# TinyMPC/tinympc-matlab

Hardware: AMD Instinct MI355X
Metric: ADMM iterations/s, batched quadrotor nx=12 nu=4 N=50 (instance-iterations/s, whole job) (higher is better)
Workload: dtype f64

## Files before the change

### __graft_entry__.py

```python
from __future__ import annotations

import hashlib
import importlib.util
import os
import re
import shutil
import subprocess
import sys

ROOT = os.path.dirname(os.path.abspath(__file__))
if ROOT not in sys.path:
    sys.path.insert(0, ROOT)
PKG_DIR = os.path.join(ROOT, "tinympc-matlab_amd")
PKG_NAME = "tinympc_matlab_amd"
CSRC = os.path.join(PKG_DIR, "csrc")
HIP_LIB = os.path.join(PKG_DIR, "libtinympc_hip.so")
ORACLE_DIR = os.path.join(ROOT, "oracle")
REFERENCE_SRC = "/root/reference/src/codegen_src"

HIP_SOURCES = ["tinympc_kernels.hip", "tinympc_precompute_rows.hip", "tinympc_solve.hip", "tinympc_solve_b.hip", "tinympc_solve_fam.hip", "tinympc_solve_adapt.hip", "tinympc_imod_a.hip", "tinympc_ifam_a.hip", "tinympc_solve_c.hip", "tinympc_solve_d.hip", "tinympc_solve_dr.hip", "tinympc_lean_d.hip", "tinympc_lstart_d.hip", "tinympc_ltrim_d.hip", "tinympc_lshare_d.hip", "tinympc_solve_dw.hip", "tinympc_solve_dx.hip", "tinympc_jit.hip", "tinympc_solve_m.hip", "tinympc_precompute_large.hip", "tinympc_handle.hip", "tinympc_plan.hip", "tinympc_session.hip", "tinympc_capi.hip",
               "tinympc_codegen.hip"]
HIP_LINTED = ["tinympc_precompute_rows.hip", "tinympc_solve.hip", "tinympc_solve_b.hip", "tinympc_solve_fam.hip", "tinympc_solve_adapt.hip", "tinympc_imod_a.hip", "tinympc_ifam_a.hip",
              "tinympc_solve_c.hip", "tinympc_solve_d.hip", "tinympc_solve_dr.hip", "tinympc_lean_d.hip", "tinympc_lstart_d.hip", "tinympc_ltrim_d.hip", "tinympc_lshare_d.hip", "tinympc_solve_dw.hip", "tinympc_solve_dx.hip"]
JIT_EMBEDDED = ["tinympc_device.h", "tinympc_sweep.h", "tinympc_fam_red.h", "tinympc_solve_d_chain.h", "tinympc_solve_dw_chain.h", "tinympc_solve_dx_chain.h",
                "tinympc_solve_e_common.h", "tinympc_solve_dwide.h", "tinympc_solve_d.hip", "tinympc_solve_dw.hip", "tinympc_solve_dx.hip", "tinympc_solve_e.hip",
                "tinympc_solve_f.hip"]
_ROCKET = ["-DTINY_JIT_NX=6", "-DTINY_JIT_NU=3", "-DTINY_JIT_N=100", "-DTINY_JIT_CT=0", "-DTINY_JIT_FAM=1"]
_ROCKET_FAM = ["-DTINY_JIT_E_NROUND=1", "-DTINY_JIT_E_NCONE=2", "-DTINY_JIT_E_CONES={0,0,2},{0,6,8}", "-DTINY_JIT_E_NLX=1", "-DTINY_JIT_E_NLU=0"]
HIP_BUILTINS = [
    ("k_builtin_e_rocket100", "tinympc_solve_e.hip",
     _ROCKET + ["-DTINY_JIT_E_WPG=8", "-DTINY_JIT_E_WPS=2", "-DTINY_JIT_E_S=13"] + _ROCKET_FAM +
     ["-DTINY_JIT_E_GC_LDS=0", "-DTINY_JIT_E_GL_LDS=0", "-DTINY_JIT_E_LX_LDS=0", "-DTINY_JIT_E_KFAM=1", "-DTINY_JIT_E_DREG=1"]),
    ("k_builtin_f_rocket100", "tinympc_solve_f.hip", _ROCKET + ["-DTINY_JIT_F_WPG=4", "-DTINY_JIT_F_S=7"] + _ROCKET_FAM + ["-DTINY_JIT_F_KFAM=1"]),
    ("k_builtin_f_rocket100_session", "tinympc_solve_f.hip", _ROCKET + ["-DTINY_JIT_F_WPG=4", "-DTINY_JIT_F_S=7"] + _ROCKET_FAM + ["-DTINY_JIT_F_KFAM=1", "-DTINY_JIT_F_SESSION=1"]),
]
_NO_FAM = ["-DTINY_JIT_E_NROUND=0", "-DTINY_JIT_E_NCONE=0", "-DTINY_JIT_E_CONES={-1,0,0}", "-DTINY_JIT_E_NLX=0", "-DTINY_JIT_E_NLU=0"]
for _name, _nx, _nu, _N, _wpg, _S in (("cartpole20", 4, 1, 20, 2, 3), ("quadrotor50", 12, 4, 50, 4, 4)):
    for _suffix, _ct, _extra in (("", 1, []), ("_var", 0, []), ("_session", 0, ["-DTINY_JIT_F_SESSION=1"])):
        HIP_BUILTINS.append(("k_builtin_f_%s%s" % (_name, _suffix), "tinympc_solve_f.hip",
                             ["-DTINY_JIT_NX=%d" % _nx, "-DTINY_JIT_NU=%d" % _nu, "-DTINY_JIT_N=%d" % _N, "-DTINY_JIT_CT=%d" % _ct, "-DTINY_JIT_FAM=0",
                              "-DTINY_JIT_F_WPG=%d" % _wpg, "-DTINY_JIT_F_S=%d" % _S] + _NO_FAM + _extra))
HIP_BUILTINS_D = [("k_builtin_d_quadrotor50_models", "tinympc_solve_d.hip",
                   ["-DTINY_JIT_NX=12", "-DTINY_JIT_NU=4", "-DTINY_JIT_N=50", "-DTINY_JIT_VREG=49", "-DTINY_JIT_WPS=1", "-DTINY_JIT_WPG=4",
                    "-DTINY_JIT_CT=1", "-DTINY_JIT_FAM=0", "-DTINY_JIT_ADAPT=0", "-DTINY_JIT_IMOD=1"]),
                  ("k_builtin_d_quadrotor20_lin1", "tinympc_solve_d.hip",
                   ["-DTINY_JIT_NX=12", "-DTINY_JIT_NU=4", "-DTINY_JIT_N=20", "-DTINY_JIT_VREG=19", "-DTINY_JIT_WPS=1", "-DTINY_JIT_WPG=4",
# ... 308 lines not shown
```

### tinympc-matlab_amd/csrc/tinympc_device.h

```cpp
#pragma once
#ifndef __HIPCC_RTC__
#include <hip/hip_runtime.h>
#endif

namespace tinympc {

__host__ __device__ inline size_t ops_doubles(int W, int KT) { return (size_t)2 * W * KT + 3 * W; }

__host__ __device__ inline size_t table_rows(int N) { return (size_t)N + 2; }

constexpr int V_PAD = 4;
__host__ __device__ inline size_t v_rows(int N) { return (size_t)N + 1 + 2 * V_PAD; }
__host__ __device__ inline size_t tables_doubles(int W, int N) { return 3 * table_rows(N) * W + W; }

#if defined(__HIPCC__) || defined(__HIPCC_RTC__)
__device__ __forceinline__ void host_store(double *p, double v) { __hip_atomic_store(p, v, __ATOMIC_RELAXED, __HIP_MEMORY_SCOPE_SYSTEM); }
#endif

struct PrecomputeParams {
    int nx, nu;
    union { double rho; const double *rho_sys; };
    const double *A, *B, *fdyn, *Qd, *Rd;
    double *Kinf, *Pinf, *Quu_inv, *AmBKt, *APf, *BPf;
    int *info;
// ... 294 lines not shown
hipError_t launch_build_inst_tables(const InstTableParams &p, hipStream_t stream);
hipError_t launch_fill_inst_models(const InstModelFillParams &p, hipStream_t stream);
hipError_t launch_store_inst_diag(const InstDiagParams &p, hipStream_t stream);
hipError_t launch_check_positive(const double *v, int n, int *flag, hipStream_t stream);
hipError_t launch_build_inst_lin(const InstLinParams &p, hipStream_t stream);
hipError_t launch_check_inst_lin(const InstLinParams &p, int *flag, hipStream_t stream);
hipError_t launch_check_inst_slopes(const InstSlopeParams &p, int *flag, hipStream_t stream);
hipError_t launch_store_inst_slopes(const InstSlopeParams &p, hipStream_t stream);
hipError_t launch_build_inst_slopes(const InstSlopeParams &p, hipStream_t stream);
hipError_t launch_check_ref_steps(const int *steps, int n, int delta, int *flag, hipStream_t stream);
hipError_t launch_advance_ref_steps(int *steps, int n, int delta, hipStream_t stream);
enum class SolveExt { Box, Families, Adaptive, InstRefs, InstBounds, InstModels, InstFamilies };
hipError_t launch_solve_a(const SolveParams &p, SolveExt ext, int W, int KT, size_t lds_bytes, hipStream_t stream);
hipError_t launch_solve_b(const SolveParams &p, int W, int KT, size_t lds_bytes, hipStream_t stream);
size_t solve_b_lds_bytes(int nx, int nu, int N, int W);
constexpr int WAVES_PER_GROUP_B = 4;
bool solve_d_supported(int nx, int nu, int N, bool const_tables);
hipError_t launch_solve_d(const SolveParams &p, hipStream_t stream);
hipError_t launch_solve_d_refill(const SolveParams &p, hipStream_t stream);
hipError_t launch_solve_d_lean(const SolveParams &p, hipStream_t stream);
hipError_t launch_solve_d_lean_start(const SolveParams &p, hipStream_t stream);
hipError_t launch_solve_d_lean_trim(const SolveParams &p, hipStream_t stream);
hipError_t launch_solve_d_lean_share(const SolveParams &p, hipStream_t stream);
int solve_d_workgroups(int nu, int N, bool const_tables, int groups);
size_t solve_d_lds_bytes(int nu, int N, bool const_tables);
int solve_d_resident_workgroups(int wpg);
int solve_d_wavefronts_per_workgroup(int nu, int N, bool const_tables);
bool solve_dw_supported(int nx, int nu, int N, bool const_tables);
hipError_t launch_solve_dw(const SolveParams &p, hipStream_t stream);
int solve_dw_workgroups(int nu, int N, int groups);
size_t solve_dw_lds_bytes(int nu, int N);
bool solve_dx_supported(int nx, int nu, int N, bool const_tables);
hipError_t launch_solve_dx(const SolveParams &p, hipStream_t stream);
int solve_dx_workgroups(int nu, int N, int groups);
size_t solve_dx_lds_bytes(int nu, int N);
hipError_t launch_solve_c(const SolveParams &p, int W, int KT, size_t lds_bytes, hipStream_t stream);
hipError_t launch_build_chunk_tables(const ChunkTableParams &p, hipStream_t stream);
size_t f_input_table_doubles(int nu, int S);
hipError_t launch_build_f_input_tables(const ChunkTableParams &p, hipStream_t stream);
void chunk_plan(int N, int *S, int *C, int *Lc);
size_t solve_c_lds_bytes(int nx, int Lc);
size_t solve_c_lds_bytes_refs(int nx, int nu, int N, int Lc);
size_t chunk_table_doubles(int nx, int Lc);
int chunk_ks(int nx);
hipError_t launch_build_adapt(const AdaptTableParams &p, hipStream_t stream);
inline hipError_t ensure_dynamic_lds(const void *fn, size_t bytes, size_t (&cache)[16]) {
// ... 42 lines not shown
```

### tinympc-matlab_amd/csrc/tinympc_plan.hip

```cpp
#include <cstring>
#include "tinympc_handle.h"

using namespace tinympc;
using namespace tinympc::host;

namespace {

void arm_completion_flag(tinympc_solver *s, SolveParams &p) {
    if (!p.host_sol) return;
    s->session_seq += 1;
    p.host_seq = (double)s->session_seq;
    s->flag_pending = true;
}

void decide_layout_d_variants(tinympc_solver *s) {
    if (!s->layout_d) return;
    if (s->d_varying < 0 && !s->tables_const()) {
        if (s->W == 16 && !s->d_jit && solve_d_supported(s->nx, s->nu, s->N, false)) {
            s->d_varying = 1;
        } else {
            s->d_varying_jit = solve_jit_supported(s->W, s->nx, s->nu, s->N, false);
            s->d_varying = s->d_varying_jit ? 1 : 0;
        }
    }
// ... 240 lines not shown
    if (pl.kernel != KernelId::D_COMPILED || s->W != 16 || pl.adaptive || pl.families || s->zero_copy_tick || s->st.max_iter <= 0)
        return false;
    if (pl.inst_models) return false;
    if (refill_applies(s, pl)) return false;
    const char *env = getenv("TINYMPC_LEAN");
    const int mode = env ? atoi(env) : -1;
    if (mode == 0) return false;
    if (mode == 1) return true;
    const bool reachable = s->st.abs_pri_tol > 0.0 && s->st.abs_dua_tol > 0.0;
    return s->st.check_termination != 1 || !reachable;
}
static bool lean_start_applies() {
    const char *env = getenv("TINYMPC_LEAN_START");
    return !env || atoi(env) != 0;
}
static bool lean_trim_applies() {
    const char *env = getenv("TINYMPC_LEAN_TRIM");
    return lean_start_applies() && (!env || atoi(env) != 0);
}
static bool lean_share_applies() {
    const char *env = getenv("TINYMPC_LEAN_SHARE");
    return lean_trim_applies() && (!env || atoi(env) != 0);
}
static const char *lean_words(const tinympc_solver *s, const LaunchPlan &pl) {
    return !lean_applies(s, pl)   ? ""
           : lean_share_applies() ? " lean lds-start trim share"
           : lean_trim_applies()  ? " lean lds-start trim"
           : lean_start_applies() ? " lean lds-start"
                                  : " lean";
}

int launch(tinympc_solver *s, bool timed) {
    int rc;
    s->flag_pending = false;
    if ((rc = resolve_plan(s))) return rc;
    const LaunchPlan pl = current_plan(s);
    const bool fam = pl.families, adaptive = pl.adaptive;
    if (s->inst.fam() && !pl.inst_lin) {
        const char *why = s->layout_m ? "for systems with nx+nu > 64"
                          : s->inst.models ? (s->inst.rho_verb ? "with per-instance models or rho (set_model_batch / set_rho_batch); tinympc_clear_model_batch returns to the shared model and rho"
                                                               : "with per-instance models (set_model_batch); tinympc_clear_model_batch returns to the shared model")
                          : adaptive ? "with adaptive rho"
                                     : "with more cones or rounds of overlapping cones than the generic kernel holds";
        if (!s->inst.lin)
            return fail(TINYMPC_ERR_UNSUPPORTED, "per-instance cone slopes (set_cone_slopes_batch) are not supported %s; "
                        "tinympc_set_cone_constraints returns to shared slopes", why);
        return fail(TINYMPC_ERR_UNSUPPORTED, "per-instance linear constraints (set_linear_constraints_batch)%s are not supported %s; "
                    "tinympc_set_linear_constraints returns to shared rows%s", s->inst.cones ? " and cone slopes (set_cone_slopes_batch)" : "", why,
// ... 97 lines not shown
    p.rho_min = s->st.adaptive_rho_min; p.rho_max = s->st.adaptive_rho_max; p.rho_clip = s->st.adaptive_rho_enable_clipping;
    const bool kernel_takes_cold = (pl.kernel == KernelId::D_COMPILED || pl.kernel == KernelId::D_JIT) && s->st.max_iter > 0;
    if (s->cold_state && !kernel_takes_cold && (rc = materialize_cold_state(s))) return rc;
    p.cold = s->cold_state ? 1 : 0;
    s->cold_state = false;
    if (s->st.max_iter > 0) s->sol_zero_pending = false;
    else if ((rc = materialize_zero_solution(s))) return rc;
    if (refill_applies(s, pl) && !p.x0_mirror && !p.u0_host && !p.host_sol) {
        if (!s->drefill && (rc = dalloc(s, &s->drefill, 1))) return rc;
        HIP_TRY(hipMemsetAsync(s->drefill, 0, sizeof(int), s->stream));
        p.refill_next = s->drefill;
    }
    if (timed) HIP_TRY(hipEventRecord(s->ev0, s->stream));
    switch (pl.kernel) {
        case KernelId::M:
            p.ctab = s->dctab;
            HIP_TRY(launch_solve_m(p, s->stream));
            break;
        case KernelId::D_JIT:
            HIP_TRY(launch_solve_jit(p, s->W, s->stream, pl.inst_models, pl.inst_lin ? s->ifam_nl() : 0, pl.inst_lin && s->inst.cones));
            break;
        case KernelId::D_COMPILED:
            if (lean_applies(s, pl) && !p.x0_mirror && !p.u0_host && !p.refill_next)
                HIP_TRY(lean_share_applies()   ? launch_solve_d_lean_share(p, s->stream)
                        : lean_trim_applies()  ? launch_solve_d_lean_trim(p, s->stream)
                        : lean_start_applies() ? launch_solve_d_lean_start(p, s->stream)
                                               : launch_solve_d_lean(p, s->stream));
            else HIP_TRY(s->W == 64 ? launch_solve_dx(p, s->stream) : s->W == 32 ? launch_solve_dw(p, s->stream) : launch_solve_d(p, s->stream));
            break;
        case KernelId::E:
            p.ctab = s->dctab_e; p.chunk_len = s->e_chunk_len; p.chunk_count = s->e_wpg; p.chunk_levels = 1;
            HIP_TRY(launch_solve_e(p, s->fs, s->stream));
            break;
        case KernelId::F:
            p.ctab = s->dctab_f; p.ftab = s->dftab; p.chunk_len = s->f_chunk_len; p.chunk_count = s->f_chunks; p.chunk_levels = 4;
            arm_completion_flag(s, p);
            HIP_TRY(launch_solve_f(p, s->f_fs, s->stream));
            break;
        case KernelId::C:
            p.ctab = s->dctab; p.chunk_len = s->chunk_len; p.chunk_count = s->chunk_count; p.chunk_levels = s->chunk_levels;
            arm_completion_flag(s, p);
            HIP_TRY(launch_solve_c(p, s->W, s->KT, s->lds_bytes_c, s->stream));
            break;
        case KernelId::B:
            HIP_TRY(launch_solve_b(p, s->W, s->KT, s->lds_bytes, s->stream));
            break;
        case KernelId::A:
// ... 107 lines not shown
```

### tinympc-matlab_amd/csrc/tinympc_solve_d.hip

```cpp
#if defined(TINY_BUILTIN) && !defined(TINY_JIT)
#define TINY_JIT 1
#endif
#ifndef TINY_JIT
#include <atomic>
#endif
#include <type_traits>

#include "tinympc_device.h"
#include "tinympc_sweep.h"

#ifndef TINY_REFILL
#if defined(TINY_JIT_REFILL) && TINY_JIT_REFILL
#define TINY_REFILL 1
#else
#define TINY_REFILL 0
#endif
#endif

#ifndef TINY_LEAN
#define TINY_LEAN 0
#endif
#if TINY_LEAN && (TINY_REFILL || defined(TINY_JIT))
#error "TINY_LEAN: compiled-in plain kernels only"
#endif
// ... 10 lines not shown
#endif
#if TINY_LEAN_START && !defined(TINY_LEAN_NO_HOIST)
#define TINY_LEAN_HOIST 1
#else
#define TINY_LEAN_HOIST 0
#endif
#ifndef TINY_LEAN_TRIM
#define TINY_LEAN_TRIM 0
#endif
#if TINY_LEAN_TRIM && !(TINY_LEAN_START && TINY_LEAN_HOIST && TINY_LDS_START)
#error "TINY_LEAN_TRIM: a variant of the lean-start kernels (LDS starts and hoisted control)"
#endif
#if TINY_LEAN_TRIM && !defined(TINY_TRIM_NO_DSTORE)
#define TINY_TRIM_DSTORE 1
#define D_DUMP_DOUBLES(nu) (2 * 4 * (nu))
#else
#define TINY_TRIM_DSTORE 0
#endif
#ifndef TINY_LEAN_SHARE
#define TINY_LEAN_SHARE 0
#endif
#if TINY_LEAN_SHARE && !(TINY_LEAN_TRIM && TINY_TRIM_DSTORE)
#error "TINY_LEAN_SHARE: a variant of the trimmed lean kernels (with their dstore addresses)"
#endif

#define TINY_STR2(x) #x
#define TINY_STR(x) TINY_STR2(x)
namespace tinympc {
template <int NX, int NU>
struct DStep;
}

#ifdef TINY_JIT
#define D_NX TINY_JIT_NX
#define D_NU TINY_JIT_NU
#include "tinympc_solve_d_chain.h"
#else
#define D_NX 12
#define D_NU 4
#include "tinympc_solve_d_chain.h"
#define D_NX 4
#define D_NU 1
#include "tinympc_solve_d_chain.h"
#endif

namespace tinympc {
// ... 232 lines not shown
    auto row_offset = [&](int i) -> unsigned { return (unsigned)(i >> 2) * (unsigned)(v_rows(N) * 64) + (unsigned)((i & 3) * 16 + r); };
#else
    double *const gV1u = p.V2 + (g0 * v_rows(N) + V_PAD) * 64;
#endif
    const unsigned voff = (unsigned)(lane + koff * 64);
    double *const sVl = sV + lane;
    const bool cold = p.cold != 0;
    if (grp_ok) {
        if (cold) {
            for (int i = lane; i < NS * DS; i += 64) sD[i] = 0.0;
            static_for<0, VL>([&](auto S) { sVl[S.value * 64] = 0.0; });
        } else {
            for (int i = lane; i < NS * DS; i += 64) sD[i] = gD[i];
            static_for<0, VL>([&](auto S) { sVl[S.value * 64] = gV0[(S.value + koff) * 64]; });
        }
    }
    __syncthreads();
    if (!grp_ok) return;
#ifdef TINY_CLOCK_STAMP
    const unsigned long long ck_barrier = __builtin_amdgcn_s_memrealtime();
#endif

    double G[NS], G0, Vr[NVR > 0 ? NVR : 1], V0;
    if (cold) {
        static_for<0, NS>([&](auto S) { G[S.value] = 0.0; });
        static_for<0, NVR>([&](auto S) { Vr[S.value] = 0.0; });
        G0 = 0.0;
        V0 = 0.0;
    } else {
        static_for<0, NS>([&](auto S) { G[S.value] = gG[(S.value + koff) * 64]; });
        static_for<0, NVR>([&](auto S) { Vr[S.value] = gV0[(VL + S.value + koff) * 64]; });
        G0 = gG[0];
        V0 = gV0[0];
    }
    double GCr[FAM ? NS : 1], GLr[FAM ? NS : 1], LX[FAM ? NS : 1], GC0 = 0.0, GL0 = 0.0;
    double cn[KT], ct_[KT], ty[KT];
    int role = 0, nl = 0;
    double mu = 0.0, inv_mu = 0.0;
    bool famc = false, faml = false, any_cone = false, any_lin = false;
    if constexpr (FAM) {
        const double *const gGC = p.GC + (g0 * v_rows(N) + V_PAD) * 64 + lane, *const gGL = p.GL + (g0 * v_rows(N) + V_PAD) * 64 + lane;
        static_for<0, NS>([&](auto S) {
            GCr[S.value] = gGC[(S.value + koff) * 64];
            GLr[S.value] = gGL[(S.value + koff) * 64];
            LX[S.value] = 0.0;
        });
// ... 137 lines not shown
                m[K.value] = fma(delta, src[o + (sAd - sOps)], src[o]);
            });
        } else {
            static_for<0, 16>([&](auto K) { m[K.value] = src[(K.value < NXU ? K.value : 0) * 16]; });
        }
    };
    auto vget = [&](auto S) -> double {
        if constexpr (decltype(S)::value >= VL) return Vr[decltype(S)::value - VL];
        else return sVl[decltype(S)::value * 64];
    };

#ifdef TINY_CLOCK_STAMP
    const unsigned long long ck_t0 = __builtin_amdgcn_s_memtime(), ck_r0 = __builtin_amdgcn_s_memrealtime();
#endif
#ifdef TINY_D_PAD
    asm volatile(".rept " TINY_STR(TINY_D_PAD) "\n\ts_nop 0\n\t.endr" ::: "memory");
#endif
#ifdef TINY_D_LOOP_ALIGN
    asm volatile(".p2align " TINY_STR(TINY_D_LOOP_ALIGN) ::: "memory");
#endif
    const int max_iter = p.max_iter;
#if TINY_TRIM_DSTORE
    unsigned aDw = aD;
#endif
#if TINY_LEAN
    auto iteration = [&](auto LEAN_, const int it) __attribute__((always_inline)) -> bool {
#if TINY_LEAN_HOIST
        constexpr bool LEANI = decltype(LEAN_)::value != 0, CTL_ONLY = decltype(LEAN_)::value == 2, NO_CTL = LEANI && !CTL_ONLY;
#if TINY_LEAN_SHARE
        constexpr bool SH_F = decltype(LEAN_)::value >= 3, SH_B = decltype(LEAN_)::value == 3;
#endif
#else
        constexpr bool LEANI = decltype(LEAN_)::value;
#endif
#else
    for (int it = 0; max_iter > 0; ++it) {
#endif
        const int it0 = __builtin_amdgcn_readfirstlane(it);
#if TINY_LEAN
        const bool final_round = !LEANI && it0 >= max_iter;
#elif TINY_REFILL
        const bool final_round = REFILL ? false : it0 >= max_iter;
#else
        const bool final_round = it0 >= max_iter;
#endif
#if TINY_LEAN_HOIST
// ... 168 lines not shown
        const bool adapt = ADAPT && __builtin_amdgcn_readfirstlane((int)((it0 > 0) && (it0 % 5 == 0))) != 0;
        double a_pr = 0.0, a_pn = 0.0, a_dr = 0.0, a_dn = 0.0;
        double gprev = 0.0;
        double mtr[16];
        if constexpr (ADAPT) {
            if (adapt) static_for<0, 16>([&](auto K) { mtr[K.value] = K.value < NXU ? sAd[2 * 256 + K.value * 16 + r] : 0.0; });
        }
        {
            const double lo0 = CT ? lo_c : sT[W + r], hi0 = CT ? hi_c : sT[TOFF + W + r];
            const double s = x0v + G0;
            const double snew = fmin(hi0, fmax(lo0, s));
#if TINY_LEAN_HOIST
            if constexpr (LEANI) G0 = s;
            else G0 = s - snew;
#else
            G0 = s - snew;
#endif
            pri = is_x ? fabs(x0v - snew) : 0.0;
            dua = is_x ? fabs(V0 - snew) : 0.0;
            if (may && !adapt) {
                const bool bad = !((pri < p.abs_pri_tol) && (dua * rho < p.abs_dua_tol));
#if TINY_REFILL
                may = __builtin_amdgcn_readfirstlane((int)wave_may_converge_d(__ballot(bad), __ballot(REFILL ? chk : active))) != 0;
#else
                may = __builtin_amdgcn_readfirstlane((int)(ILIN ? wave_may_converge_d32(__ballot(bad), __ballot(active)) : wave_may_converge_d(__ballot(bad), __ballot(active)))) != 0;
#endif
            }
#if TINY_REFILL
            if (TINY_RARE(may) && is_x && active) gV1u[REFILL ? row_offset(cur) : (unsigned)lane] = V0;
#else
            if (TINY_RARE(may) && is_x && active) gV1u[(unsigned)lane] = V0;
#endif
            V0 = snew;
        }
        if constexpr (FAM) {
            double gcn, gln;
            (void)families(x0v, GC0, GL0, gcn, gln);
            if (is_x) {
                GC0 = gcn;
                GL0 = gln;
            }
        }
        double xcur = x0v;
#if TINY_LEAN_SHARE
        double dcur = 0.0, vcur = 0.0;
        if constexpr (!(SH_F && VL == 0)) dcur = lds_read_async<0>(aD);
#else
        double dcur = lds_read_async<0>(aD), vcur = 0.0;
#endif
#if TINY_LEAN
        if constexpr (VL > 0 && !LEANI) vcur = lds_read_async<0>(aV);
#else
        if constexpr (VL > 0) vcur = lds_read_async<0>(aV);
#endif
        double locur = lo_c, hicur = hi_c;
        if constexpr (!CT) {
            locur = lds_read_async<W * 8>(aT);
            hicur = lds_read_async<(TOFF + W) * 8>(aT);
        }
        lds_wait_ops(m);
#if TINY_LDS_START
        double acur = 0.0;
#endif
        auto fstep = [&](auto S) {
            constexpr int q = decltype(S)::value;
            double dn = 0.0, vn = 0.0, lon = lo_c, hin = hi_c;
#if TINY_LEAN_SHARE
            if constexpr (q + 1 < NS && !(SH_F && q + 1 >= VL)) dn = lds_read_async<(q + 1) * DS * 8>(aD);
#else
            if constexpr (q + 1 < NS) dn = lds_read_async<(q + 1) * DS * 8>(aD);
#endif
#if TINY_LEAN
            if constexpr (q + 1 < VL && !LEANI) vn = lds_read_async<(q + 1) * 512>(aV);
#else
            if constexpr (q + 1 < VL) vn = lds_read_async<(q + 1) * 512>(aV);
#endif
            if constexpr (!CT && q + 1 < NS) {
                lon = lds_read_async<(q + 2) * W * 8>(aT);
                hin = lds_read_async<(TOFF + (q + 2) * W) * 8>(aT);
            }
#if TINY_LDS_START
            static_assert(K0, "step 0 starts from c0");
            double an = 0.0;
            if constexpr (LEANI && q + 1 < NS) an = lds_read_issued_here<0>(aC);
#endif
            const double xprev = xcur;
            double snew_q;
#if TINY_LEAN
            if constexpr (LEANI) {
                if constexpr (q >= VL) {
#if TINY_LEAN_SHARE
                    if constexpr (SH_F && K0 && q == 0) xcur = Step::fwd_reg0_nores(Vr[q - VL], m, c0, locur, hicur, G[q], Vr[q - VL]);
                    else if constexpr (SH_F) xcur = Step::fwd_reg_start(xcur, Vr[q - VL], m, acur, locur, hicur, G[q], Vr[q - VL]);
                    else
#endif
                    if constexpr (K0 && q == 0) xcur = Step::fwd_reg0_nores(dcur, m, c0, locur, hicur, G[q], Vr[q - VL]);
#if TINY_LDS_START
                    else xcur = Step::fwd_reg_start(xcur, dcur, m, acur, locur, hicur, G[q], Vr[q - VL]);
#else
                    else xcur = Step::fwd_reg_nores(xcur, dcur, m, cf, locur, hicur, G[q], Vr[q - VL]);
#endif
                    snew_q = Vr[q - VL];
                } else {
                    double vnew;
                    if constexpr (K0 && q == 0) xcur = Step::fwd_lds0_nores(dcur, m, c0, locur, hicur, G[q], vnew);
#if TINY_LDS_START
                    else xcur = Step::fwd_lds_start(xcur, dcur, m, acur, locur, hicur, G[q], vnew);
#else
                    else xcur = Step::fwd_lds_nores(xcur, dcur, m, cf, locur, hicur, G[q], vnew);
#endif
                    lds_write_async<q * 512>(aV, vnew);
                    snew_q = vnew;
// ... 34 lines not shown
                }
            }
            dcur = dn;
            vcur = vn;
#if TINY_LDS_START
            acur = an;
#endif
            if constexpr (!CT) {
                locur = lon;
                hicur = hin;
            }
        };
        constexpr int DF = D_FIRST < NS ? D_FIRST : NS;
        constexpr int NG = 1 + (NS - DF + D_GROUP - 1) / D_GROUP;
        static_for<0, NG>([&](auto Gi) {
            constexpr int s0 = Gi.value == 0 ? 0 : DF + (Gi.value - 1) * D_GROUP;
            constexpr int s1 = Gi.value == 0 ? DF : ((s0 + D_GROUP < NS) ? s0 + D_GROUP : NS);
            if (TINY_RARE(may)) {
                if constexpr (s0 > 0) {
                    if (!adapt) {
                        const bool bad = !((pri < p.abs_pri_tol) && (dua * rho < p.abs_dua_tol));
#if TINY_REFILL
                        may = __builtin_amdgcn_readfirstlane((int)wave_may_converge_d(__ballot(bad), __ballot(REFILL ? chk : active))) != 0;
#else
                        may = __builtin_amdgcn_readfirstlane((int)(ILIN ? wave_may_converge_d32(__ballot(bad), __ballot(active)) : wave_may_converge_d(__ballot(bad), __ballot(active)))) != 0;
#endif
                    }
                }
                if (TINY_RARE(may)) {
#if TINY_REFILL
                    unsigned vo = REFILL ? row_offset(cur) + (unsigned)(koff * 64) : voff;
#else
                    unsigned vo = voff;
#endif
                    double *base = gV1u;
                    asm volatile("" : "+v"(vo), "+s"(base));
                    if (active) static_for<s0, s1>([&](auto S) { (base + S.value * 64)[vo] = vget(S); });
                }
            }
            static_for<s0, s1>([&](auto S) { fstep(S); });
        });
#if TINY_REFILL
        if constexpr (REFILL) {
            if (active) it_done += 1;
        } else {
            if (active) it_done = it1;
        }
#elif TINY_LEAN_HOIST
        if constexpr (!NO_CTL) {
            if (active) it_done = it1;
        }
#else
        if (active) it_done = it1;
#endif

        const double nrho_lin = nrho, rhom_lin = rhom, pnref_lin = pnref;
        if constexpr (ADAPT) {
            if (adapt) {
                const double x_last = xcur, g_last = gprev;
                double pr[16];
                const double delta = rho - rho0;
                static_for<0, 16>([&](auto K) {
                    constexpr int o = K.value * 16;
                    pr[K.value] = K.value < NXU ? fma(delta, sAd[4 * 256 + o + r], sAd[3 * 256 + o + r]) : 0.0;
                });
                const double pxl = group_matvec<W, 16>(pr, is_x ? x_last : 0.0, 0.0);
                if (is_x) {
                    const double qv = dgr * x_last;
                    a_dn = fmax(fmax(fmax(a_dn, fabs(pxl)), fabs(qv)), fabs(g_last));
                    a_dr = fmax(a_dr, fabs(pxl + qv - g_last));
                }
                const double pri_res = group_max<W>(a_pr), pri_norm = group_max<W>(a_pn);
                const double dual_res = group_max<W>(a_dr), dual_norm = group_max<W>(a_dn);
                const double eps = 1e-10;
                const double normalized_pri = pri_res / (pri_norm + eps);
                const double normalized_dual = dual_res / (dual_norm + eps);
// ... 78 lines not shown
                        : [v1] "v"(v1), [g1] "v"(G[NS - 1]), [v2] "v"(v2), [g2] "v"(G[NS - 2]), [nrho] "v"(nrho_lin), [lrT] "v"(lrT),
                          [rhom] "v"(rhom_lin), [lrmc] "v"(lrmc2), [lr] "v"(lr2));
                } else if constexpr (FOLD) {
                    asm("v_add_f64 %[t], %[v1], -%[g1]\n\t"
                        "v_fma_f64 %[px], %[sc], %[t], %[lrT]\n\t"
                        "v_add_f64 %[rn], %[v2], -%[g2]\n\t"
                        "v_fma_f64 %[acc], %[rhom], %[rn], %[lrmc]"
                        : [t] "=&v"(t), [px] "=&v"(px), [acc] "=&v"(acc), [rn] "=&v"(rnext)
                        : [v1] "v"(v1), [g1] "v"(G[NS - 1]), [v2] "v"(v2), [g2] "v"(G[NS - 2]), [sc] "v"(is_x ? nrho : 1.0),
                          [lrT] "v"(is_x ? pnref : 0.0), [rhom] "v"(rhom), [lrmc] "v"(lrmc_f));
                } else {
                    asm("v_add_f64 %[t], %[v1], -%[g1]\n\t"
                        "v_fma_f64 %[px], %[nrho], %[t], %[lrT]\n\t"
                        "v_add_f64 %[t], %[v2], -%[g2]\n\t"
                        "v_fma_f64 %[acc], %[rhom], %[t], %[lrmc]\n\t"
                        "v_fma_f64 %[rn], %[nrho], %[t], %[lr]"
                        : [t] "=&v"(t), [px] "=&v"(px), [acc] "=&v"(acc), [rn] "=&v"(rnext)
                        : [v1] "v"(v1), [g1] "v"(G[NS - 1]), [v2] "v"(v2), [g2] "v"(G[NS - 2]), [nrho] "s"(nrho), [lrT] "v"(lrT),
                          [rhom] "v"(rhom), [lrmc] "v"(lrmc2), [lr] "v"(lr2));
                }
                rcur = px;
            }
            auto vreq = [&](auto S) -> double {
                if constexpr (decltype(S)::value >= VL) return Vr[decltype(S)::value - VL];
                else return lds_read_async<decltype(S)::value * 512>(aV);
            };
            double v2cur = vreq(std::integral_constant<int, (NS >= 3 ? NS - 3 : 0)>{});
            lds_wait_ops(m);
#if TINY_LEAN_HOIST
            if constexpr (LEANI) {
                asm volatile("" : "+v"(G0));
                G0 = G0 - V0;
                asm volatile("" ::"v"(G0));
            }
#endif
            static_for<0, NS - 1>([&](auto I) {
                constexpr int s = NS - 1 - I.value;
                constexpr int s2 = s >= 2 ? s - 2 : 0;
                constexpr int s3 = s >= 3 ? s - 3 : 0;
                double v2n = 0.0;
                if constexpr (s >= 2) v2n = vreq(std::integral_constant<int, s3>{});
                const double lr2 = lr_of(std::integral_constant<int, s2>{});
                const double lrmc2 = is_x ? lr2 + cb : cb;
#if TINY_LEAN_SHARE
                if constexpr (SH_B && s >= VL) {
                    constexpr bool AN_REG = s - 1 >= VL;
                    double &an_s = Vr[AN_REG ? s - 1 - VL : 0];
                    double an_l, rn;
                    const double v2op = (s == 1 && AN_REG) ? rhom : v2cur;
                    if constexpr (FOLD && AN_REG) Step::bwd_fold(Vr[s - VL], px, rcur, m, v2op, G[s2], rhom, lrmc_f, an_s, rn);
                    else if constexpr (FOLD) Step::bwd_fold(Vr[s - VL], px, rcur, m, v2op, G[s2], rhom, lrmc_f, an_l, rn);
                    else if constexpr (AN_REG) Step::bwd(Vr[s - VL], px, rcur, m, v2op, G[s2], rhom, lrmc2, nrho, lr2, an_s, rn);
                    else Step::bwd(Vr[s - VL], px, rcur, m, v2op, G[s2], rhom, lrmc2, nrho, lr2, an_l, rn);
                    if constexpr (!AN_REG) acc = an_l;
                    px = Vr[s - VL];
                    rcur = rnext;
                    rnext = rn;
                    v2cur = v2n;
                    return;
                }
#endif
                double a = acc, an, rn;
                if constexpr (ADAPT) Step::bwd_v(a, px, rcur, m, v2cur, G[s2], rhom_lin, lrmc2, nrho_lin, lr2, an, rn);
                else if constexpr (FOLD) Step::bwd_fold(a, px, rcur, m, v2cur, G[s2], rhom, lrmc_f, an, rn);
                else Step::bwd(a, px, rcur, m, v2cur, G[s2], rhom, lrmc2, nrho, lr2, an, rn);
#if TINY_TRIM_DSTORE
                if constexpr (NO_CTL) lds_write_async<s * DS * 8>(aDw, a);
// ... 29 lines not shown
    const int last_check = ct > 0 ? (max_iter / ct) * ct : 0;
    for (int it = 0; max_iter > 0;) {
        int nres = max_iter + 1;
        if (ct > 0 && reachable) nres = (it / ct + 1) * ct;
        else if (last_check > it) nres = last_check;
        const int lean_end = __builtin_amdgcn_readfirstlane(nres - 1 < max_iter ? nres - 1 : max_iter);
#if TINY_LEAN_HOIST
        if (it < lean_end) {
            if (iteration(std::integral_constant<int, 2>{}, it)) break;
#if TINY_TRIM_DSTORE
            {
                const unsigned long long live = __ballot(active);
                const unsigned lm = (unsigned)(live & 1ull) | (unsigned)((live >> 15) & 2ull) | (unsigned)((live >> 30) & 4ull) | (unsigned)((live >> 45) & 8ull);
                const int first = __builtin_ctz(lm | 16u);
                const int cls = (r / NU) % 3;
                int jt = cls == 0 ? j : (j ^ 2);
                if (((lm >> jt) & 1u) == 0u) jt = first & 3;
                const unsigned dump = lds_addr(sD) + (unsigned)((jt * NU + r % NU) * 8) - (unsigned)((cls == 2 ? 2 : 1) * DS * 8);
                aDw = (is_u && active) ? aD : dump;
            }
#endif
#if TINY_LEAN_SHARE
            static_for<0, NVR>([&](auto S) { Vr[S.value] = lds_read_async<(VL + S.value) * DS * 8>(aD); });
            lds_wait();
            static_for<0, NVR>([&](auto S) {
                double &vr = Vr[decltype(S)::value];
                asm volatile("" : "+v"(vr));
            });
            for (; it < lean_end - 1; ++it) (void)iteration(std::integral_constant<int, 3>{}, it);
            (void)iteration(std::integral_constant<int, 4>{}, it);
            ++it;
#else
            for (; it < lean_end; ++it) (void)iteration(std::true_type{}, it);
#endif
            if (active) it_done = __builtin_amdgcn_readfirstlane(it);
        }
        if (iteration(std::false_type{}, it)) break;
#else
        bool over = false;
        for (; it < lean_end; ++it) {
            if (iteration(std::true_type{}, it)) {
                over = true;
                break;
            }
        }
        if (over || iteration(std::false_type{}, it)) break;
#endif
// ... 15 lines not shown
        const int rows = is_x ? N : NS;
        double *const wV = p.V + ((size_t)grp * v_rows(N) + V_PAD) * 64 + lane;
        const double *const wV2 = p.V2 + ((size_t)grp * v_rows(N) + V_PAD) * 64 + lane;
        for (int kn = 0; kn < rows; ++kn) wV[kn * 64] = wV2[kn * 64];
    }

    const double res_px = group_max<W>(is_x ? snap_pri : 0.0), res_pu = group_max<W>(is_u ? snap_pri : 0.0);
    const double rho_res = ADAPT ? snap_rho : rho;
    const double res_dx = group_max<W>(is_x ? snap_dua : 0.0) * rho_res, res_du = group_max<W>(is_u ? snap_dua : 0.0) * rho_res;

#ifdef TINY_CLOCK_STAMP
    if (p.scratch && lane == 0) {
        unsigned long long *ck = reinterpret_cast<unsigned long long *>(p.scratch) + 8 * (size_t)grp;
        ck[0] = ck_t1 - ck_t0;
        ck[1] = ck_r1 - ck_r0;
        ck[2] = ck_barrier - ck_entry;
        ck[3] = ck_r0 - ck_barrier;
        ck[4] = __builtin_amdgcn_s_memrealtime() - ck_r1;
        ck[5] = ck_entry;
        ck[6] = __builtin_amdgcn_s_memrealtime();
        ck[7] = (unsigned long long)__builtin_amdgcn_s_getreg((31 << 11) | 4) | ((unsigned long long)__builtin_amdgcn_s_getreg((3 << 11) | 20) << 32);
    }
#endif
    if (inst_ok && r == 0) {
        if constexpr (ADAPT) p.rho_inst[inst] = rho;
        p.istats[inst * 2 + 0] = it_done;
        p.istats[inst * 2 + 1] = status;
        if (res_valid) {
            p.dstats[inst * 4 + 0] = res_px;
            p.dstats[inst * 4 + 1] = res_dx;
            p.dstats[inst * 4 + 2] = res_pu;
            p.dstats[inst * 4 + 3] = res_du;
        }
    }
}

#if TINY_LEAN
#if TINY_LEAN_SHARE
#define k_admm_solve_d_lean k_admm_solve_d_lean_share
#define k_admm_solve_d_gbnd_lean k_admm_solve_d_gbnd_lean_share
#define launch_solve_d_lean launch_solve_d_lean_share
static_assert(d_vl(4, 50, true, 4) == 25, "quadrotor N=50: 25 slack slots in LDS with four wavefronts per workgroup");
#elif TINY_LEAN_TRIM
#define k_admm_solve_d_lean k_admm_solve_d_lean_trim
#define k_admm_solve_d_gbnd_lean k_admm_solve_d_gbnd_lean_trim
#define launch_solve_d_lean launch_solve_d_lean_trim
static_assert(d_vl(4, 50, true, 4) == 25, "quadrotor N=50: 25 slack slots in LDS with four wavefronts per workgroup");
#elif TINY_LEAN_START
#define k_admm_solve_d_lean k_admm_solve_d_lean_start
#define k_admm_solve_d_gbnd_lean k_admm_solve_d_gbnd_lean_start
#define launch_solve_d_lean launch_solve_d_lean_start
static_assert(d_vl(4, 50, true, 4) == 25, "quadrotor N=50: 25 slack slots in LDS with four wavefronts per workgroup");
#endif
template <int NX, int NU, int N, bool CT, int WPG, int VL>
__global__ void __launch_bounds__(64 * WPG) __attribute__((amdgpu_waves_per_eu(2, 2))) k_admm_solve_d_lean(const SolveParams p) {
    extern __shared__ __attribute__((aligned(16))) double smem[];
    k_admm_solve_d_body<NX, NU, N, CT, WPG, VL>(p, smem);
}
template <int NX, int NU, int N, int WPG, int VL>
__global__ void __launch_bounds__(64 * WPG) __attribute__((amdgpu_waves_per_eu(2, 2))) k_admm_solve_d_gbnd_lean(const SolveParams p) {
    extern __shared__ __attribute__((aligned(16))) double smem[];
// ... 13 lines not shown
        static size_t lds_set_l[16] = {0}, lds_set_lgoal[16] = {0};
        const int wgs = (p.groups + WPG - 1) / WPG;
        if (p.x0_mirror || p.u0_host || p.refill_next) return hipErrorInvalidValue;
        if (p.iref_pn) {
            if constexpr (!CT) {
                return hipErrorInvalidValue;
            } else {
                if (!p.iref_lr || !p.ibnd) return hipErrorInvalidValue;
                auto fn = &k_admm_solve_d_gbnd_lean<NX, NU, N, WPG, VL>;
                hipError_t e = ensure_dynamic_lds(reinterpret_cast<const void *>(fn), lds, lds_set_lgoal);
                if (e != hipSuccess) return e;
                hipLaunchKernelGGL(fn, dim3(wgs), dim3(64 * WPG), lds, stream, p);
            }
        } else {
            auto fn = &k_admm_solve_d_lean<NX, NU, N, CT, WPG, VL>;
            hipError_t e = ensure_dynamic_lds(reinterpret_cast<const void *>(fn), lds, lds_set_l);
            if (e != hipSuccess) return e;
            hipLaunchKernelGGL(fn, dim3(wgs), dim3(64 * WPG), lds, stream, p);
        }
        return hipGetLastError();
    }
}

hipError_t launch_solve_d_lean(const SolveParams &p, hipStream_t stream) {
    if (p.nx == 12 && p.nu == 4 && p.N == 50) return p.const_tables ? launch_d_one<12, 4, 50, true>(p, stream) : launch_d_one<12, 4, 50, false>(p, stream);
    if (p.nx == 4 && p.nu == 1 && p.N == 20) return p.const_tables ? launch_d_one<4, 1, 20, true>(p, stream) : launch_d_one<4, 1, 20, false>(p, stream);
    if (p.nx == 4 && p.nu == 1 && p.N == 10) return p.const_tables ? launch_d_one<4, 1, 10, true>(p, stream) : launch_d_one<4, 1, 10, false>(p, stream);
    return hipErrorInvalidValue;
}
#else
#ifndef TINY_JIT
#if TINY_REFILL
template <int NX, int NU, int N, bool CT, int WPG, int VL>
__global__ void __launch_bounds__(64 * WPG) __attribute__((amdgpu_waves_per_eu(2, 2))) k_admm_solve_d_refill(const SolveParams p) {
#else
template <int NX, int NU, int N, bool CT, int WPG, int VL, bool HOSTX = false>
__global__ void __launch_bounds__(64 * WPG) __attribute__((amdgpu_waves_per_eu(2, 2))) k_admm_solve_d(const SolveParams p) {
#endif
    extern __shared__ __attribute__((aligned(16))) double smem[];
#if TINY_REFILL
    k_admm_solve_d_body<NX, NU, N, CT, WPG, VL, false, false, true, false, true>(p, smem);
#else
    k_admm_solve_d_body<NX, NU, N, CT, WPG, VL, false, false, true, HOSTX>(p, smem);
#endif
}
#if !TINY_REFILL
template <int NX, int NU, int N, int WPG, int VL>
__global__ void __launch_bounds__(64 * WPG) __attribute__((amdgpu_waves_per_eu(2, 2))) k_admm_solve_d_gbnd(const SolveParams p) {
    extern __shared__ __attribute__((aligned(16))) double smem[];
    k_admm_solve_d_body<NX, NU, N, true, WPG, VL, false, false, true, false, false, true>(p, smem);
}
#endif
// ... 190 lines not shown
```

Before: 1.192 billion.

## Add park variant of lean solve kernel moving slack slots from LDS to registers

Adds a new lean-share kernel variant in which 12 of the LDS-resident slack slots are held in registers (Vx) instead. To free registers for them, the convergence snapshot and status are parked in the LDS space those slots vacate during the run and restored afterwards. It is selected by default for quadrotor N=50 with constant tables when the run length allows it, and can be disabled with an environment variable. It trades more register pressure, plus extra park/unpark LDS traffic, for fewer LDS reads and writes in the forward and backward sweeps.

```diff
diff --git a/__graft_entry__.py b/__graft_entry__.py
--- a/__graft_entry__.py
+++ b/__graft_entry__.py
@@ -18,10 +18,10 @@
 ORACLE_DIR = os.path.join(ROOT, "oracle")
 REFERENCE_SRC = "/root/reference/src/codegen_src"
 
-HIP_SOURCES = ["tinympc_kernels.hip", "tinympc_precompute_rows.hip", "tinympc_solve.hip", "tinympc_solve_b.hip", "tinympc_solve_fam.hip", "tinympc_solve_adapt.hip", "tinympc_imod_a.hip", "tinympc_ifam_a.hip", "tinympc_solve_c.hip", "tinympc_solve_d.hip", "tinympc_solve_dr.hip", "tinympc_lean_d.hip", "tinympc_lstart_d.hip", "tinympc_ltrim_d.hip", "tinympc_lshare_d.hip", "tinympc_solve_dw.hip", "tinympc_solve_dx.hip", "tinympc_jit.hip", "tinympc_solve_m.hip", "tinympc_precompute_large.hip", "tinympc_handle.hip", "tinympc_plan.hip", "tinympc_session.hip", "tinympc_capi.hip",
+HIP_SOURCES = ["tinympc_kernels.hip", "tinympc_precompute_rows.hip", "tinympc_solve.hip", "tinympc_solve_b.hip", "tinympc_solve_fam.hip", "tinympc_solve_adapt.hip", "tinympc_imod_a.hip", "tinympc_ifam_a.hip", "tinympc_solve_c.hip", "tinympc_solve_d.hip", "tinympc_solve_dr.hip", "tinympc_lean_d.hip", "tinympc_lstart_d.hip", "tinympc_ltrim_d.hip", "tinympc_lshare_d.hip", "tinympc_lpark_d.hip", "tinympc_solve_dw.hip", "tinympc_solve_dx.hip", "tinympc_jit.hip", "tinympc_solve_m.hip", "tinympc_precompute_large.hip", "tinympc_handle.hip", "tinympc_plan.hip", "tinympc_session.hip", "tinympc_capi.hip",
                "tinympc_codegen.hip"]
 HIP_LINTED = ["tinympc_precompute_rows.hip", "tinympc_solve.hip", "tinympc_solve_b.hip", "tinympc_solve_fam.hip", "tinympc_solve_adapt.hip", "tinympc_imod_a.hip", "tinympc_ifam_a.hip",
-              "tinympc_solve_c.hip", "tinympc_solve_d.hip", "tinympc_solve_dr.hip", "tinympc_lean_d.hip", "tinympc_lstart_d.hip", "tinympc_ltrim_d.hip", "tinympc_lshare_d.hip", "tinympc_solve_dw.hip", "tinympc_solve_dx.hip"]
+              "tinympc_solve_c.hip", "tinympc_solve_d.hip", "tinympc_solve_dr.hip", "tinympc_lean_d.hip", "tinympc_lstart_d.hip", "tinympc_ltrim_d.hip", "tinympc_lshare_d.hip", "tinympc_lpark_d.hip", "tinympc_solve_dw.hip", "tinympc_solve_dx.hip"]
 JIT_EMBEDDED = ["tinympc_device.h", "tinympc_sweep.h", "tinympc_fam_red.h", "tinympc_solve_d_chain.h", "tinympc_solve_dw_chain.h", "tinympc_solve_dx_chain.h",
                 "tinympc_solve_e_common.h", "tinympc_solve_dwide.h", "tinympc_solve_d.hip", "tinympc_solve_dw.hip", "tinympc_solve_dx.hip", "tinympc_solve_e.hip",
                 "tinympc_solve_f.hip"]
diff --git a/tinympc-matlab_amd/csrc/tinympc_device.h b/tinympc-matlab_amd/csrc/tinympc_device.h
--- a/tinympc-matlab_amd/csrc/tinympc_device.h
+++ b/tinympc-matlab_amd/csrc/tinympc_device.h
@@ -340,6 +340,7 @@
 hipError_t launch_solve_d_lean_start(const SolveParams &p, hipStream_t stream);
 hipError_t launch_solve_d_lean_trim(const SolveParams &p, hipStream_t stream);
 hipError_t launch_solve_d_lean_share(const SolveParams &p, hipStream_t stream);
+hipError_t launch_solve_d_lean_park(const SolveParams &p, hipStream_t stream);
 int solve_d_workgroups(int nu, int N, bool const_tables, int groups);
 size_t solve_d_lds_bytes(int nu, int N, bool const_tables);
 int solve_d_resident_workgroups(int wpg);
diff --git a/tinympc-matlab_amd/csrc/tinympc_lpark_d.hip b/tinympc-matlab_amd/csrc/tinympc_lpark_d.hip
--- /dev/null
+++ b/tinympc-matlab_amd/csrc/tinympc_lpark_d.hip
@@ -0,0 +1,6 @@
+#define TINY_LEAN 1
+#define TINY_LEAN_START 1
+#define TINY_LEAN_TRIM 1
+#define TINY_LEAN_SHARE 1
+#define TINY_LEAN_PARK 1
+#include "tinympc_solve_d.hip"
diff --git a/tinympc-matlab_amd/csrc/tinympc_plan.hip b/tinympc-matlab_amd/csrc/tinympc_plan.hip
--- a/tinympc-matlab_amd/csrc/tinympc_plan.hip
+++ b/tinympc-matlab_amd/csrc/tinympc_plan.hip
@@ -286,8 +286,24 @@
     const char *env = getenv("TINYMPC_LEAN_SHARE");
     return lean_trim_applies() && (!env || atoi(env) != 0);
 }
+constexpr int PARK_MIN_RUN = 6;
+static int first_lean_run(const tinympc_solver *s) {
+    const int max_iter = s->st.max_iter, ct = s->st.check_termination;
+    const bool reachable = s->st.abs_pri_tol > 0.0 && s->st.abs_dua_tol > 0.0;
+    if (ct > 0 && reachable) return ct - 1 < max_iter ? ct - 1 : max_iter;
+    const int last_check = ct > 0 ? (max_iter / ct) * ct : 0;
+    return last_check > 0 ? last_check - 1 : max_iter;
+}
+static bool lean_park_applies(const tinympc_solver *s) {
+    const char *env = getenv("TINYMPC_LEAN_PARK");
+    if (!lean_share_applies() || (env && atoi(env) == 0)) return false;
+    if (!(s->nx == 12 && s->nu == 4 && s->N == 50)) return false;
+    return first_lean_run(s) >= PARK_MIN_RUN;
+}
 static const char *lean_words(const tinympc_solver *s, const LaunchPlan &pl) {
+    const bool ct = s->tables_const() || (pl.inst_refs && pl.kernel != KernelId::A);
     return !lean_applies(s, pl)   ? ""
+           : ct && lean_park_applies(s) ? " lean lds-start trim share park"
            : lean_share_applies() ? " lean lds-start trim share"
            : lean_trim_applies()  ? " lean lds-start trim"
            : lean_start_applies() ? " lean lds-start"
@@ -431,7 +447,8 @@
             break;
         case KernelId::D_COMPILED:
             if (lean_applies(s, pl) && !p.x0_mirror && !p.u0_host && !p.refill_next)
-                HIP_TRY(lean_share_applies()   ? launch_solve_d_lean_share(p, s->stream)
+                HIP_TRY(p.const_tables && lean_park_applies(s) ? launch_solve_d_lean_park(p, s->stream)
+                        : lean_share_applies() ? launch_solve_d_lean_share(p, s->stream)
                         : lean_trim_applies()  ? launch_solve_d_lean_trim(p, s->stream)
                         : lean_start_applies() ? launch_solve_d_lean_start(p, s->stream)
                                                : launch_solve_d_lean(p, s->stream));
diff --git a/tinympc-matlab_amd/csrc/tinympc_solve_d.hip b/tinympc-matlab_amd/csrc/tinympc_solve_d.hip
--- a/tinympc-matlab_amd/csrc/tinympc_solve_d.hip
+++ b/tinympc-matlab_amd/csrc/tinympc_solve_d.hip
@@ -56,6 +56,15 @@
 #endif
 #if TINY_LEAN_SHARE && !(TINY_LEAN_TRIM && TINY_TRIM_DSTORE)
 #error "TINY_LEAN_SHARE: a variant of the trimmed lean kernels (with their dstore addresses)"
+#endif
+#ifndef TINY_LEAN_PARK
+#define TINY_LEAN_PARK 0
+#endif
+#if TINY_LEAN_PARK && !TINY_LEAN_SHARE
+#error "TINY_LEAN_PARK: a variant of the shared lean kernels"
+#endif
+#if TINY_LEAN_PARK && !defined(TINY_PARK_SLOTS)
+#define TINY_PARK_SLOTS 12
 #endif
 
 #define TINY_STR2(x) #x
@@ -334,6 +343,11 @@
 #endif
 
     double G[NS], G0, Vr[NVR > 0 ? NVR : 1], V0;
+#if TINY_LEAN_PARK
+    static_assert(VL > TINY_PARK_SLOTS && TINY_PARK_SLOTS > 0, "the converted slots are LDS slots, and slot 0 stays one");
+    constexpr int VLR = VL - TINY_PARK_SLOTS, NVX = VL - VLR;
+    double Vx[NVX];
+#endif
     if (cold) {
         static_for<0, NS>([&](auto S) { G[S.value] = 0.0; });
         static_for<0, NVR>([&](auto S) { Vr[S.value] = 0.0; });
@@ -517,6 +531,26 @@
     const int max_iter = p.max_iter;
 #if TINY_TRIM_DSTORE
     unsigned aDw = aD;
+#endif
+#if TINY_LEAN_PARK
+    constexpr int PARK_ROWS = 3;
+    static_assert(PARK_ROWS * 64 <= (NS - VLR) * DS, "the parked rows fit into the d rows of the run's register slots");
+    auto park = [&]() __attribute__((always_inline)) {
+        const unsigned aP = lds_addr(sD + VLR * DS + lane);
+        lds_write_async<0 * 512>(aP, snap_pri);
+        lds_write_async<1 * 512>(aP, snap_dua);
+        lds_write_async<2 * 512>(aP, __hiloint2double(status, it_done));
+    };
+    auto unpark = [&]() __attribute__((always_inline)) {
+        const unsigned aP = lds_addr(sD + VLR * DS + lane);
+        double p0 = lds_read_async<0 * 512>(aP), p1 = lds_read_async<1 * 512>(aP), p2 = lds_read_async<2 * 512>(aP);
+        lds_wait();
+        asm volatile("" : "+v"(p0), "+v"(p1), "+v"(p2));
+        snap_pri = p0;
+        snap_dua = p1;
+        status = __double2hiint(p2);
+        it_done = __double2loint(p2);
+    };
 #endif
 #if TINY_LEAN
     auto iteration = [&](auto LEAN_, const int it) __attribute__((always_inline)) -> bool {
@@ -731,12 +765,21 @@
                 const bool bad = !((pri < p.abs_pri_tol) && (dua * rho < p.abs_dua_tol));
 #if TINY_REFILL
                 may = __builtin_amdgcn_readfirstlane((int)wave_may_converge_d(__ballot(bad), __ballot(REFILL ? chk : active))) != 0;
+#elif TINY_LEAN_PARK
+                may = __builtin_amdgcn_readfirstlane((int)wave_may_converge_d32(__ballot(bad), __ballot(active))) != 0;
 #else
                 may = __builtin_amdgcn_readfirstlane((int)(ILIN ? wave_may_converge_d32(__ballot(bad), __ballot(active)) : wave_may_converge_d(__ballot(bad), __ballot(active)))) != 0;
 #endif
             }
 #if TINY_REFILL
             if (TINY_RARE(may) && is_x && active) gV1u[REFILL ? row_offset(cur) : (unsigned)lane] = V0;
+#elif TINY_LEAN_PARK
+            if (TINY_RARE(may) && is_x && active) {
+                unsigned lo = (unsigned)lane;
+                double *base = gV1u;
+                asm volatile("" : "+v"(lo), "+s"(base));
+                base[lo] = V0;
+            }
 #else
             if (TINY_RARE(may) && is_x && active) gV1u[(unsigned)lane] = V0;
 #endif
@@ -751,7 +794,9 @@
             }
         }
         double xcur = x0v;
-#if TINY_LEAN_SHARE
+#if TINY_LEAN_PARK
+        double dcur = lds_read_async<0>(aD), vcur = 0.0;
+#elif TINY_LEAN_SHARE
         double dcur = 0.0, vcur = 0.0;
         if constexpr (!(SH_F && VL == 0)) dcur = lds_read_async<0>(aD);
 #else
@@ -774,7 +819,9 @@
         auto fstep = [&](auto S) {
             constexpr int q = decltype(S)::value;
             double dn = 0.0, vn = 0.0, lon = lo_c, hin = hi_c;
-#if TINY_LEAN_SHARE
+#if TINY_LEAN_PARK
+            if constexpr (q + 1 < NS && !(SH_F && q + 1 >= VLR)) dn = lds_read_async<(q + 1) * DS * 8>(aD);
+#elif TINY_LEAN_SHARE
             if constexpr (q + 1 < NS && !(SH_F && q + 1 >= VL)) dn = lds_read_async<(q + 1) * DS * 8>(aD);
 #else
             if constexpr (q + 1 < NS) dn = lds_read_async<(q + 1) * DS * 8>(aD);
@@ -797,6 +844,19 @@
             double snew_q;
 #if TINY_LEAN
             if constexpr (LEANI) {
+#if TINY_LEAN_PARK
+                if constexpr (SH_F && q >= VLR && q < VL) {
+                    if constexpr (SH_B) {
+                        xcur = Step::fwd_reg_start(xcur, Vx[q - VLR], m, acur, locur, hicur, G[q], Vx[q - VLR]);
+                        snew_q = Vx[q - VLR];
+                    } else {
+                        double vnew;
+                        xcur = Step::fwd_lds_start(xcur, Vx[q - VLR], m, acur, locur, hicur, G[q], vnew);
+                        lds_write_async<q * 512>(aV, vnew);
+                        snew_q = vnew;
+                    }
+                } else
+#endif
                 if constexpr (q >= VL) {
 #if TINY_LEAN_SHARE
                     if constexpr (SH_F && K0 && q == 0) xcur = Step::fwd_reg0_nores(Vr[q - VL], m, c0, locur, hicur, G[q], Vr[q - VL]);
@@ -877,6 +937,8 @@
                         const bool bad = !((pri < p.abs_pri_tol) && (dua * rho < p.abs_dua_tol));
 #if TINY_REFILL
                         may = __builtin_amdgcn_readfirstlane((int)wave_may_converge_d(__ballot(bad), __ballot(REFILL ? chk : active))) != 0;
+#elif TINY_LEAN_PARK
+                        may = __builtin_amdgcn_readfirstlane((int)wave_may_converge_d32(__ballot(bad), __ballot(active))) != 0;
 #else
                         may = __builtin_amdgcn_readfirstlane((int)(ILIN ? wave_may_converge_d32(__ballot(bad), __ballot(active)) : wave_may_converge_d(__ballot(bad), __ballot(active)))) != 0;
 #endif
@@ -907,6 +969,9 @@
         }
 #else
         if (active) it_done = it1;
+#endif
+#if TINY_LEAN_PARK
+        if constexpr (SH_F && !SH_B) unpark();
 #endif
 
         const double nrho_lin = nrho, rhom_lin = rhom, pnref_lin = pnref;
@@ -1031,6 +1096,10 @@
                 rcur = px;
             }
             auto vreq = [&](auto S) -> double {
+#if TINY_LEAN_PARK
+                if constexpr (SH_B && decltype(S)::value >= VLR && decltype(S)::value < VL) return Vx[decltype(S)::value - VLR];
+                else
+#endif
                 if constexpr (decltype(S)::value >= VL) return Vr[decltype(S)::value - VL];
                 else return lds_read_async<decltype(S)::value * 512>(aV);
             };
@@ -1051,7 +1120,24 @@
                 if constexpr (s >= 2) v2n = vreq(std::integral_constant<int, s3>{});
                 const double lr2 = lr_of(std::integral_constant<int, s2>{});
                 const double lrmc2 = is_x ? lr2 + cb : cb;
-#if TINY_LEAN_SHARE
+#if TINY_LEAN_PARK
+                if constexpr (SH_B && s >= VLR) {
+                    constexpr bool AN_REG = s - 1 >= VLR;
+                    constexpr int sn = AN_REG ? s - 1 : s;
+                    double &a_s = s >= VL ? Vr[s >= VL ? s - VL : 0] : Vx[s >= VL ? 0 : s - VLR];
+                    double &an_s = sn >= VL ? Vr[sn >= VL ? sn - VL : 0] : Vx[sn >= VL ? 0 : sn - VLR];
+                    double an_l, rn;
+                    static_assert(FOLD, "constant tables only");
+                    if constexpr (AN_REG) Step::bwd_fold(a_s, px, rcur, m, v2cur, G[s2], rhom, lrmc_f, an_s, rn);
+                    else Step::bwd_fold(a_s, px, rcur, m, v2cur, G[s2], rhom, lrmc_f, an_l, rn);
+                    if constexpr (!AN_REG) acc = an_l;
+                    px = a_s;
+                    rcur = rnext;
+                    rnext = rn;
+                    v2cur = v2n;
+                    return;
+                }
+#elif TINY_LEAN_SHARE
                 if constexpr (SH_B && s >= VL) {
                     constexpr bool AN_REG = s - 1 >= VL;
                     double &an_s = Vr[AN_REG ? s - 1 - VL : 0];
@@ -1127,7 +1213,17 @@
 #endif
 #if TINY_LEAN_SHARE
             static_for<0, NVR>([&](auto S) { Vr[S.value] = lds_read_async<(VL + S.value) * DS * 8>(aD); });
+#if TINY_LEAN_PARK
+            static_for<0, NVX>([&](auto S) { Vx[S.value] = lds_read_async<(VLR + S.value) * DS * 8>(aD); });
             lds_wait();
+            static_for<0, NVX>([&](auto S) {
+                double &vx = Vx[decltype(S)::value];
+                asm volatile("" : "+v"(vx));
+            });
+            park();
+#else
+            lds_wait();
+#endif
             static_for<0, NVR>([&](auto S) {
                 double &vr = Vr[decltype(S)::value];
                 asm volatile("" : "+v"(vr));
@@ -1189,6 +1285,21 @@
         ck[7] = (unsigned long long)__builtin_amdgcn_s_getreg((31 << 11) | 4) | ((unsigned long long)__builtin_amdgcn_s_getreg((3 << 11) | 20) << 32);
     }
 #endif
+#if TINY_LEAN_PARK
+    int lane_e = lane;
+    asm volatile("" : "+v"(lane_e));
+    const long inst_e = grp * IPW + (lane_e >> 4);
+    if (inst_ok && r == 0) {
+        p.istats[inst_e * 2 + 0] = it_done;
+        p.istats[inst_e * 2 + 1] = status;
+        if (res_valid) {
+            p.dstats[inst_e * 4 + 0] = res_px;
+            p.dstats[inst_e * 4 + 1] = res_dx;
+            p.dstats[inst_e * 4 + 2] = res_pu;
+            p.dstats[inst_e * 4 + 3] = res_du;
+        }
+    }
+#else
     if (inst_ok && r == 0) {
         if constexpr (ADAPT) p.rho_inst[inst] = rho;
         p.istats[inst * 2 + 0] = it_done;
@@ -1200,10 +1311,16 @@
             p.dstats[inst * 4 + 3] = res_du;
         }
     }
+#endif
 }
 
 #if TINY_LEAN
-#if TINY_LEAN_SHARE
+#if TINY_LEAN_PARK
+#define k_admm_solve_d_lean k_admm_solve_d_lean_park
+#define k_admm_solve_d_gbnd_lean k_admm_solve_d_gbnd_lean_park
+#define launch_solve_d_lean launch_solve_d_lean_park
+static_assert(d_vl(4, 50, true, 4) == 25, "quadrotor N=50: 25 slack slots in LDS with four wavefronts per workgroup");
+#elif TINY_LEAN_SHARE
 #define k_admm_solve_d_lean k_admm_solve_d_lean_share
 #define k_admm_solve_d_gbnd_lean k_admm_solve_d_gbnd_lean_share
 #define launch_solve_d_lean launch_solve_d_lean_share
@@ -1263,12 +1380,19 @@
     }
 }
 
+#if TINY_LEAN_PARK
+hipError_t launch_solve_d_lean(const SolveParams &p, hipStream_t stream) {
+    if (p.nx == 12 && p.nu == 4 && p.N == 50 && p.const_tables) return launch_d_one<12, 4, 50, true>(p, stream);
+    return hipErrorInvalidValue;
+}
+#else
 hipError_t launch_solve_d_lean(const SolveParams &p, hipStream_t stream) {
     if (p.nx == 12 && p.nu == 4 && p.N == 50) return p.const_tables ? launch_d_one<12, 4, 50, true>(p, stream) : launch_d_one<12, 4, 50, false>(p, stream);
     if (p.nx == 4 && p.nu == 1 && p.N == 20) return p.const_tables ? launch_d_one<4, 1, 20, true>(p, stream) : launch_d_one<4, 1, 20, false>(p, stream);
     if (p.nx == 4 && p.nu == 1 && p.N == 10) return p.const_tables ? launch_d_one<4, 1, 10, true>(p, stream) : launch_d_one<4, 1, 10, false>(p, stream);
     return hipErrorInvalidValue;
 }
+#endif
 #else
 #ifndef TINY_JIT
 #if TINY_REFILL
```

Result: faster. 1.208 billion, median of 6 (+1.3%).
